# miuda-ai/lele

Hardware: AMD Instinct MI355X
Metric: STFT+mel GB/s (SenseVoice front-end: PCM -> log-mel -> LFR, algorithmic bytes); SenseVoiceSmall-shaped RTF in `sensevoice` (higher is better)
Workload: dtype f32

## Files before the change

lele_amd/csrc/fe_core.h:

```cpp
#pragma once
#include <stdint.h>

#if defined(__HIPCC__)
#define FE_HD __host__ __device__ __forceinline__
#else
#define FE_HD inline
#endif

namespace fe {

constexpr int kNfft = 512;
constexpr int kFrame = 400;
constexpr int kHop = 160;
constexpr int kBins = 257;
constexpr int kLanes = 16;
constexpr int kRegs = 32;
constexpr int kQ = 25;

FE_HD constexpr int rev4(int x) { return ((x & 1) << 3) | ((x & 2) << 1) | ((x & 4) >> 1) | ((x & 8) >> 3); }
FE_HD constexpr int rev5(int x) {
    return ((x & 1) << 4) | ((x & 2) << 2) | (x & 4) | ((x & 8) >> 2) | ((x & 16) >> 4);
}
FE_HD constexpr int tw_off(int s) { return (1 << (s - 1)) - 1; }

FE_HD float fmul(float a, float b) { return a * b; }
FE_HD float fadd(float a, float b) { return a + b; }
FE_HD float fsub(float a, float b) { return a - b; }
FE_HD float ffma(float a, float b, float c) { return __builtin_fmaf(a, b, c); }

#if defined(__HIPCC__) && defined(__HIP_DEVICE_COMPILE__)
typedef float cf __attribute__((ext_vector_type(2)));
FE_HD cf cmk(float re, float im) { return (cf){re, im}; }
FE_HD cf cadd(cf a, cf b) { return a + b; }
FE_HD cf csub(cf a, cf b) { return a - b; }
FE_HD cf cmulv(cf a, cf b) { return a * b; }
FE_HD cf cfmav(cf a, cf b, cf c) { return __builtin_elementwise_fma(a, b, c); }
FE_HD cf cswap(cf a) { return a.yx; }
FE_HD cf cxx(cf a) { return a.xx; }
#else
struct cf {
    float x, y;
};
FE_HD cf cmk(float re, float im) { return cf{re, im}; }
FE_HD cf cadd(cf a, cf b) { return cf{a.x + b.x, a.y + b.y}; }
FE_HD cf csub(cf a, cf b) { return cf{a.x - b.x, a.y - b.y}; }
FE_HD cf cmulv(cf a, cf b) { return cf{a.x * b.x, a.y * b.y}; }
FE_HD cf cfmav(cf a, cf b, cf c) { return cf{__builtin_fmaf(a.x, b.x, c.x), __builtin_fmaf(a.y, b.y, c.y)}; }
FE_HD cf cswap(cf a) { return cf{a.y, a.x}; }
FE_HD cf cxx(cf a) { return cf{a.x, a.x}; }
#endif

struct Tw {
    cf w, wn;
};
FE_HD Tw make_tw(float wr, float wi) { return Tw{cmk(wr, wi), cmk(-wi, wi)}; }

FE_HD cf tw_mul_fma(const Tw& t, cf o) { return cfmav(cxx(t.w), o, cmulv(t.wn, cswap(o))); }

FE_HD void bfly_fma(const Tw& tw, cf& e, cf& o) {
    cf t = tw_mul_fma(tw, o);
    cf n = csub(e, t);
    e = cadd(e, t);
    o = n;
}
FE_HD void bfly_scalar(float wr, float wi, cf& e, cf& o) {
    float tr = fsub(fmul(wr, o.x), fmul(wi, o.y));
    float ti = fadd(fmul(wr, o.y), fmul(wi, o.x));
    cf t = cmk(tr, ti);
    cf n = csub(e, t);
    e = cadd(e, t);
    o = n;
}
FE_HD void bfly_fma(float wr, float wi, float& er, float& ei, float& o_r, float& oi) {
    cf e = cmk(er, ei), o = cmk(o_r, oi);
    bfly_fma(make_tw(wr, wi), e, o);
    er = e.x;
    ei = e.y;
    o_r = o.x;
    oi = o.y;
}
FE_HD void bfly_scalar(float wr, float wi, float& er, float& ei, float& o_r, float& oi) {
    cf e = cmk(er, ei), o = cmk(o_r, oi);
    bfly_scalar(wr, wi, e, o);
    er = e.x;
    ei = e.y;
    o_r = o.x;
    oi = o.y;
}

template <typename TW>
FE_HD void phase_a(cf* a, const TW& tw_re, const TW& tw_im) {
#pragma unroll
    for (int r = 0; r < kRegs; r += 2) bfly_scalar(tw_re[tw_off(1)], tw_im[tw_off(1)], a[r], a[r + 1]);
#pragma unroll
    for (int b = 0; b < kRegs; b += 4) {
#pragma unroll
        for (int k = 0; k < 2; ++k) bfly_scalar(tw_re[tw_off(2) + k], tw_im[tw_off(2) + k], a[b + k], a[b + 2 + k]);
    }
#pragma unroll
    for (int s = 3; s <= 5; ++s) {
        const int half = 1 << (s - 1);
#pragma unroll
        for (int b = 0; b < kRegs; b += 2 * half) {
#pragma unroll
            for (int k = 0; k < half; ++k)
                bfly_fma(make_tw(tw_re[tw_off(s) + k], tw_im[tw_off(s) + k]), a[b + k], a[b + half + k]);
        }
    }
}

template <typename TW>
FE_HD void phase_a_fast(const float* x, cf* a, const TW& tw_re, const TW& tw_im) {
    float s1[kRegs];
#pragma unroll
    for (int r = 0; r < kRegs; r += 2) {
        if (rev5(r + 1) >= kQ) {
            s1[r] = x[r];
            s1[r + 1] = x[r];
        } else {
            s1[r] = fadd(x[r], x[r + 1]);
            s1[r + 1] = fsub(x[r], x[r + 1]);
        }
    }
    {
        const float wr = tw_re[tw_off(2) + 1], wi = tw_im[tw_off(2) + 1];
#pragma unroll
        for (int b = 0; b < kRegs; b += 4) {
            a[b] = cmk(fadd(s1[b], s1[b + 2]), 0.0f);
            a[b + 2] = cmk(fsub(s1[b], s1[b + 2]), 0.0f);
            const float tr = fmul(wr, s1[b + 3]);
            const float ti = fmul(wi, s1[b + 3]);
            a[b + 1] = cmk(fadd(s1[b + 1], tr), ti);
            a[b + 3] = cmk(fsub(s1[b + 1], tr), -ti);
        }
    }
#pragma unroll
    for (int b = 0; b < kRegs; b += 8) {
#pragma unroll
        for (int k = 0; k < 4; ++k) {
            const float wr = tw_re[tw_off(3) + k], wi = tw_im[tw_off(3) + k];
            if ((k & 1) == 0) {
                const float e = a[b + k].x, o = a[b + 4 + k].x;
                const float tr = fmul(wr, o);
                const float ti = fmul(wi, o);
                a[b + k] = cmk(fadd(e, tr), ti);
                a[b + 4 + k] = cmk(fsub(e, tr), -ti);
            } else {
                bfly_fma(make_tw(wr, wi), a[b + k], a[b + 4 + k]);
            }
        }
    }
#pragma unroll
    for (int s = 4; s <= 5; ++s) {
        const int half = 1 << (s - 1);
#pragma unroll
        for (int b = 0; b < kRegs; b += 2 * half) {
#pragma unroll
            for (int k = 0; k < half; ++k)
                bfly_fma(make_tw(tw_re[tw_off(s) + k], tw_im[tw_off(s) + k]), a[b + k], a[b + half + k]);
        }
    }
}

template <typename TWF>
FE_HD void phase_b(cf* b, int c, int rho, const TWF& twf, float* re256) {
#pragma unroll
    for (int s = 6; s <= 8; ++s) {
        const int hv = 1 << (s - 6);
#pragma unroll
        for (int k = 0; k < hv; ++k) {
            const cf w = twf(tw_off(s) + k * 32 + rho * 16 + c);
            const Tw tw = make_tw(w.x, w.y);
#pragma unroll
            for (int base = 0; base < 16; base += 2 * hv) bfly_fma(tw, b[base + k], b[base + hv + k]);
        }
    }
#pragma unroll
    for (int k = 0; k < 8; ++k) {
        const cf w = twf(tw_off(9) + k * 32 + rho * 16 + c);
        const cf t = tw_mul_fma(make_tw(w.x, w.y), b[8 + k]);
        if (k == 0) *re256 = fsub(b[0].x, t.x);
        b[k] = cadd(b[k], t);
    }
}

FE_HD float power(float re, float im) { return fadd(fmul(re, re), fmul(im, im)); }
FE_HD float power(cf z) {
    cf sq = cmulv(z, z);
    return fadd(sq.x, sq.y);
}

constexpr int kXchgPitch = 17;
FE_HD constexpr int xchg_slot(int v, int c) { return v * kXchgPitch + c; }

}
```

lele_amd/csrc/frontend.hip:

```cpp
#include <type_traits>
#include "common.h"
#include "fe_core.h"

#include <math.h>

#include <algorithm>

using namespace lele;

namespace {

constexpr int kMaxMelRounds = 8;

struct FeDev {
    const float* tw_re;
    const float* tw_im;
    const float2* tw;
    const float* window;
    const float* melw;
    const int* mel_start;
    const int* mel_step_off;
    int mel_rounds;
    int mel_steps;
    int n_mels;
// ... 97 lines not shown

__device__ __forceinline__ const float* fe_const_table(const float* t, int pass) {
    auto c = (const __attribute__((address_space(4))) float*)t;
    asm("" : "+s"(c) : "s"(pass));
    return (const float*)c;
}

template <int MODE>
__device__ __forceinline__ float lane_rot_prev(float v, int p) {
    if (MODE == 1) {
        return __builtin_bit_cast(float,
                                  __builtin_amdgcn_update_dpp(0, __builtin_bit_cast(int, v), 0x121, 0xf, 0xf, true));
    } else {
        return __shfl(v, (p + 15) & 15, 16);
    }
}

constexpr int kStdMelLen[5] = {3, 4, 6, 10, 17};
constexpr int kStdMelOff[6] = {0, 3, 7, 13, 23, 40};

template <int MODE, bool STDMEL, bool FUSED, int PASSES, bool LOWREG, class Blk>
__device__ __forceinline__ void fe_main_body(const float* __restrict__ pcm, int64_t utt_stride,
                                             int64_t num_frames, int64_t t_lfr,
                                             const float* __restrict__ means, const FeDev& tb,
                                             float* __restrict__ out, float* __restrict__ logmel_out,
                                             int aligned16, float* s_melw, Blk bl) {
    constexpr int FR = 16 * PASSES;
    constexpr int kRows = FR + 2;
    constexpr int kXFloats = FUSED ? (kRows * kSumPitch > 4 * kWaveLdsFloats ? kRows * kSumPitch : 4 * kWaveLdsFloats)
                                   : 4 * kWaveLdsFloats;
    __shared__ float2 s_tw[LOWREG ? 480 : 512];
    __shared__ __attribute__((aligned(16))) float s_x[kXFloats];
    __shared__ float s_mean[64];
    __shared__ int s_mstart[16 * (STDMEL ? 5 : kMaxMelRounds)];
    __shared__ int s_moff[kMaxMelRounds + 1];
    constexpr int kTwBase = LOWREG ? 31 : 0;

    const int lane = threadIdx.x & 63, wave = threadIdx.x >> 6;
    const int g = lane >> 4, p = lane & 15;
    constexpr int kVecPerRow = fe::kHop / 4;
    constexpr int kVecs = kRows * kVecPerRow;
    constexpr int kIters = (kVecs + 255) / 256;
    constexpr bool kTwDma = FUSED && !LOWREG;
    const bool tile_dma = FUSED && !LOWREG && aligned16 && tb.tile_dma;
    float4 st[FUSED ? kIters : 1];
    if constexpr (FUSED) {
        const float* run = pcm + (int64_t)bl.y() * utt_stride + (int64_t)bl.x() * FR * fe::kHop;
        const int64_t rem64 = utt_stride - (int64_t)bl.x() * FR * fe::kHop;
        const int rem = (int)(rem64 < (1 << 20) ? rem64 : (1 << 20));
        if (tile_dma) {
            constexpr int kSlotsPerRow = kSumPitch / 4;
            constexpr int kDma = (FR - 1 + 2) * kSlotsPerRow + (fe::kFrame - 2 * fe::kHop) / 4;
            constexpr int kDmaInstr = (kDma + 63) / 64;
            static_assert(kDmaInstr * 64 * 4 <= kXFloats, "the tile DMA stays inside s_x");
            auto* tile_lds = (__attribute__((address_space(3))) char*)s_x;
            static_assert(kSlotsPerRow == 41 && kDmaInstr * 64 * 1599 < (1 << 24), "i / 41 == (i * 1599) >> 16 for every slot");
            const unsigned last = 4u * (unsigned)rem - 16u;
            const int wave_s = __builtin_amdgcn_readfirstlane(wave);
#pragma unroll
            for (int u = 0; 4 * u < kDmaInstr; ++u) {
                const unsigned i = 256u * u + threadIdx.x;
                const unsigned ob = 16u * (i - ((i * 1599u) >> 16));
                if (4 * u + 3 < kDmaInstr || 4 * u + wave_s < kDmaInstr)
                    fe_dma16(reinterpret_cast<const char*>(run) + (ob < last ? ob : last), tile_lds + (4 * u + wave_s) * 1024);
            }
        }
        if (kTwDma && wave == 3) {
            auto* tw_lds = (__attribute__((address_space(3))) char*)s_tw;
#pragma unroll
            for (int k = 0; k < 4; ++k)
                fe_dma16(reinterpret_cast<const char*>(tb.tw) + 1024 * k + 16 * lane, tw_lds + 1024 * k);
        }
        if (!tile_dma) {
#pragma unroll
            for (int u = 0; u < kIters; ++u) {
                const int idx = u * 256 + (int)threadIdx.x;
                int o = 4 * idx;
                if (o + 3 >= rem) o = aligned16 ? ((rem - 4) & ~3) : (rem - 4);
                const float* src = run + o;
                if (aligned16)
                    st[u] = *reinterpret_cast<const float4*>(src);
                else
                    st[u] = make_float4(src[0], src[1], src[2], src[3]);
            }
        }
    }
    if (!kTwDma)
        for (int i = threadIdx.x; i < 511 - kTwBase; i += 256) s_tw[i] = tb.tw[i + kTwBase];
    if (!STDMEL)
        for (int i = threadIdx.x; i < tb.mel_steps * 16; i += 256) s_melw[i] = tb.melw[i];
    if (threadIdx.x < tb.mel_rounds * 16) s_mstart[threadIdx.x] = tb.mel_start[threadIdx.x];
    if (threadIdx.x <= tb.mel_rounds) s_moff[threadIdx.x] = tb.mel_step_off[threadIdx.x];
    if (FUSED) {
        if (!tile_dma) {
#pragma unroll
            for (int u = 0; u < kIters; ++u) {
                const int idx = u * 256 + (int)threadIdx.x;
                if (idx < kVecs) {
                    const int row = idx / kVecPerRow, c = idx - row * kVecPerRow;
                    *reinterpret_cast<float4*>(&s_x[row * kSumPitch + 4 * c]) = st[u];
                }
            }
        }
        __builtin_amdgcn_s_waitcnt(0x0F70);
        __syncthreads();
    }
    const int h = fe::rev4(p);
    float* xw = s_x + wave * kWaveLdsFloats;
    float* xf = xw + g * kFrameXchgFloats;
    const float* base = pcm + (int64_t)bl.y() * utt_stride;
    const float* mean_u = means + (int64_t)bl.y() * num_frames;
    const int d_out = tb.n_mels * tb.lfr_m;
    float* out_u = out ? out + (int64_t)bl.y() * t_lfr * d_out : nullptr;
    float* lm_u = logmel_out ? logmel_out + (int64_t)bl.y() * num_frames * tb.n_mels : nullptr;

    float win[fe::kQ];
    if (!LOWREG) {
#pragma unroll
        for (int q = 0; q < fe::kQ; ++q) win[q] = tb.window[p + 16 * q];
    }

    float xr[fe::kQ];
    float mean_next = 0.0f;
    auto issue_loads = [&](int pass) {
        const int64_t f = (int64_t)bl.x() * FR + wave * (4 * PASSES) + pass * 4 + g;
        const int64_t fc = f < num_frames ? f : 0;
        const float* src = base + fc * fe::kHop + p;
        if (!FUSED) mean_next = mean_u[fc];
#pragma unroll
        for (int q = 0; q < fe::kQ; ++q) xr[q] = src[16 * q];
    };
    issue_loads(0);
    if (FUSED) {
        if (wave == 0 && lane < FR) {
            float sum = 0.0f;
#pragma unroll
            for (int seg = 0; seg < 3; ++seg) {
                const float* rowp = &s_x[(lane + seg) * kSumPitch];
                const int nvec = seg < 2 ? kVecPerRow : (fe::kFrame - 2 * fe::kHop) / 4;
#pragma unroll 10
                for (int k = 0; k < nvec; ++k) {
                    const float4 r = *reinterpret_cast<const float4*>(rowp + 4 * k);
                    sum = __builtin_fmaf(r.x, 32768.0f, sum);
                    sum = __builtin_fmaf(r.y, 32768.0f, sum);
                    sum = __builtin_fmaf(r.z, 32768.0f, sum);
                    sum = __builtin_fmaf(r.w, 32768.0f, sum);
                }
            }
            s_mean[lane] = sum / (float)fe::kFrame;
        }
    }
    __syncthreads();

    auto run_pass = [&](int pass, auto load_next_c) {
        constexpr bool load_next = decltype(load_next_c)::value;
        const int64_t f = (int64_t)bl.x() * FR + wave * (4 * PASSES) + pass * 4 + g;
        const bool valid = f < num_frames;
        const float mean = FUSED ? s_mean[wave * (4 * PASSES) + pass * 4 + g] : mean_next;
        if (LOWREG) {
            int off = 0;
            asm volatile("" : "+v"(off));
#pragma unroll
            for (int q = 0; q < fe::kQ; ++q) win[q] = tb.window[p + 16 * q + off];
        }

        float v[fe::kQ];
        const float neg_mean = -mean;
#pragma unroll
        for (int q = 0; q < fe::kQ; ++q) v[q] = __builtin_fmaf(xr[q], 32768.0f, neg_mean);
        if (load_next) issue_loads(pass + 1);
        float xin[fe::kRegs];
#pragma unroll
        for (int r = 0; r < fe::kRegs; ++r) xin[r] = 0.0f;
        float k97;
        asm("v_mov_b32 %0, 0x3f7851ec" : "=v"(k97));
#pragma unroll
        for (int q = 0; q < fe::kQ; ++q) {
            const float send = (p == 15 && q > 0) ? v[q > 0 ? q - 1 : 0] : v[q];
            const float prev = lane_rot_prev<MODE>(send, p);
            float y = fe::fsub(v[q], fe::fmul(k97, prev));
            if (q == 0) y = (p == 0) ? v[0] : y;
            xin[fe::rev5(q)] = fe::fmul(y, win[q]);
        }

        fe::cf a[fe::kRegs];
        fe::phase_a_fast(xin, a, fe_const_table(tb.tw_re, pass), fe_const_table(tb.tw_im, pass));

        float pw[2][8];
        float p256 = 0.0f;
#pragma unroll
        for (int rho = 0; rho < 2; ++rho) {
            __builtin_amdgcn_wave_barrier();
#pragma unroll
            for (int cc = 0; cc < 16; ++cc) {
                const int slot = fe::xchg_slot(h, cc);
                *reinterpret_cast<float2*>(xf + 2 * slot) = make_float2(a[rho * 16 + cc].x, a[rho * 16 + cc].y);
            }
            __builtin_amdgcn_wave_barrier();
            fe::cf bq[16];
#pragma unroll
            for (int vv = 0; vv < 16; ++vv) {
                const float2 t = *reinterpret_cast<const float2*>(xf + 2 * fe::xchg_slot(vv, p));
                bq[vv] = fe::cmk(t.x, t.y);
            }
            __builtin_amdgcn_wave_barrier();
            float re256 = 0.0f;
            fe::phase_b(bq, p, rho, [&](int i) { const float2 w = s_tw[i - kTwBase]; return fe::cmk(w.x, w.y); }, &re256);
            if (rho == 0) p256 = re256;
#pragma unroll
            for (int vv = 0; vv < 8; ++vv) {
                fe::cf z = bq[vv];
                if (vv == 0 && rho == 0) z = fe::cmk(z.x, (p == 0) ? 0.0f : z.y);
                pw[rho][vv] = fe::power(z);
            }
        }
        float* prow = xw + g * kPStride;
        __builtin_amdgcn_wave_barrier();
#pragma unroll
        for (int rho = 0; rho < 2; ++rho)
#pragma unroll
            for (int vv = 0; vv < 8; ++vv) prow[(2 * vv + rho) * 16 + p] = pw[rho][vv];
        if (p == 0) prow[256] = fe::power(p256, 0.0f);
        __builtin_amdgcn_wave_barrier();

        const int fi = (int)f, nfr = (int)num_frames, tl = (int)t_lfr;
        const int pad = (tb.lfr_m - 1) / 2;
        const int fp = fi + pad;
        const int b_first = fp % tb.lfr_n, i_first = fp / tb.lfr_n;

        float vals[STDMEL ? 5 : kMaxMelRounds];
#pragma unroll
        for (int rd = 0; rd < (STDMEL ? 5 : kMaxMelRounds); ++rd) {
            vals[rd] = 0.0f;
            if (!STDMEL && rd >= tb.mel_rounds) continue;
            const int m = rd * 16 + p;
            const int start = s_mstart[m];
            const float* pp = prow + start;
            float acc = 0.0f;
            if (STDMEL) {
                const float* wp = tb.melw + kStdMelOff[rd < 5 ? rd : 0] * 16 + p;
                float w[17];
#pragma unroll
                for (int t = 0; t < 17; ++t)
                    if (t < kStdMelLen[rd < 5 ? rd : 0]) w[t] = wp[t * 16];
#pragma unroll
                for (int t = 0; t < 17; ++t)
                    if (t < kStdMelLen[rd < 5 ? rd : 0]) acc = fe::fadd(acc, fe::fmul(w[t], pp[t]));
            } else {
                const int t0 = s_moff[rd], t1 = s_moff[rd + 1];
                const float* wp = s_melw + t0 * 16 + p;
                const int lim = 256 - start;
#pragma unroll 4
                for (int t = 0; t < t1 - t0; ++t) {
                    const float pv = pp[t < lim ? t : lim];
                    acc = fe::fadd(acc, fe::fmul(wp[t * 16], pv));
                }
            }
            {
                const float l2 = __builtin_amdgcn_logf(fmaxf(acc, 1e-5f));
                const float hi = __builtin_bit_cast(float, 0x3f317217u), lo = __builtin_bit_cast(float, 0x3377d1cfu);
                const float r = fe::fmul(l2, hi);
                vals[rd] = fe::fadd(r, fe::ffma(l2, lo, fe::ffma(l2, hi, -r)));
            }
        }
        if (valid) {
            constexpr int kR = STDMEL ? 5 : kMaxMelRounds;
            auto put = [&](float* dst) {
#pragma unroll
                for (int rd = 0; rd < kR; ++rd)
                    if (rd * 16 + p < tb.n_mels) __builtin_nontemporal_store(vals[rd], &dst[rd * 16]);
            };
            if (lm_u) put(lm_u + (int64_t)fi * tb.n_mels + p);
            if (out_u) {
                int i = i_first;
                for (int b = b_first; b < tb.lfr_m && i >= 0; b += tb.lfr_n, --i)
                    if (i < tl) put(out_u + i * d_out + b * tb.n_mels + p);
                if (fi == 0) {
                    for (int i2 = 0; i2 * tb.lfr_n - pad < 0 && i2 < tl; ++i2)
                        for (int b = 0; b < tb.lfr_m && i2 * tb.lfr_n + b - pad < 0; ++b)
                            put(out_u + i2 * d_out + b * tb.n_mels + p);
                }
                if (fi == nfr - 1) {
                    for (int i2 = tl - 1; i2 >= 0 && i2 * tb.lfr_n + (tb.lfr_m - 1) - pad > fi; --i2)
                        for (int b = tb.lfr_m - 1; b >= 0 && i2 * tb.lfr_n + b - pad > fi; --b)
                            put(out_u + i2 * d_out + b * tb.n_mels + p);
                }
            }
        }
        __builtin_amdgcn_wave_barrier();
    };
#pragma unroll 1
    for (int pass = 0; pass + 1 < PASSES; ++pass) run_pass(pass, std::true_type{});
    run_pass(PASSES - 1, std::false_type{});
}

template <int MODE, bool STDMEL, bool FUSED>
__global__ __launch_bounds__(256) void fe_main_kernel(const float* __restrict__ pcm, int64_t utt_stride, int64_t num_frames, int64_t t_lfr,
                                                      const float* __restrict__ means, FeDev tb, float* __restrict__ out,
                                                      float* __restrict__ logmel_out, int aligned16) {
    extern __shared__ float s_melw[];
    fe_main_body<MODE, STDMEL, FUSED, 4, false>(pcm, utt_stride, num_frames, t_lfr, means, tb, out, logmel_out, aligned16, s_melw,
                                                GridBlock{});
}

template <int MODE, bool STDMEL>
__global__ __launch_bounds__(256) void fe_seg_main_kernel(const float* __restrict__ pcm, const FeSeg* __restrict__ segs,
                                                          const int* __restrict__ blk_seg, FeDev tb, float* __restrict__ out) {
    extern __shared__ float s_melw[];
    const FeSeg s = segs[blk_seg[blockIdx.x]];
    const float* base = pcm + s.start;
    const int aligned16 = (((uintptr_t)base & 15) == 0) && (s.len % 4 == 0);
    fe_main_body<MODE, STDMEL, true, 4, false>(base, s.len, s.num_frames, s.t_lfr, nullptr, tb, out + s.row0 * (tb.n_mels * tb.lfr_m),
                                               nullptr, aligned16, s_melw, SegBlock{(unsigned)(blockIdx.x - s.block0)});
}
__global__ void fe_generic_mean_kernel(const float* __restrict__ pcm, int64_t rows, int64_t num_frames, int64_t pcm_len, int frame_len, int hop,
                                       float* __restrict__ mean) {
    const int64_t f = (int64_t)blockIdx.x * blockDim.x + threadIdx.x;
    if (f >= rows) return;
    const float* src = pcm + (f / num_frames) * pcm_len + (f % num_frames) * hop;
    float sum = 0.0f;
    int j = 0;
    if ((((uintptr_t)src) & 15) == 0) {
        for (; j + 16 <= frame_len; j += 16) {
            float4 v[4];
#pragma unroll
            for (int u = 0; u < 4; ++u) v[u] = *reinterpret_cast<const float4*>(src + j + 4 * u);
#pragma unroll
            for (int u = 0; u < 4; ++u) {
                sum = sum + v[u].x * 32768.0f;
                sum = sum + v[u].y * 32768.0f;
                sum = sum + v[u].z * 32768.0f;
                sum = sum + v[u].w * 32768.0f;
            }
        }
    }
    for (; j < frame_len; ++j) sum = sum + src[j] * 32768.0f;
    mean[f] = sum / (float)frame_len;
}
__global__ void fe_generic_frame_kernel(const float* __restrict__ pcm, const float* __restrict__ mean,
                                        const float* __restrict__ window, int64_t rows, int64_t num_frames, int64_t pcm_len, int frame_len, int hop,
                                        int n_fft, float* __restrict__ frames) {
    const int64_t total = rows * n_fft;
    for (int64_t i = (int64_t)blockIdx.x * blockDim.x + threadIdx.x; i < total; i += (int64_t)gridDim.x * blockDim.x) {
        const int64_t f = i / n_fft;
        const int j = (int)(i - f * n_fft);
        float v = 0.0f;
        if (j < frame_len) {
            const float* src = pcm + (f / num_frames) * pcm_len + (f % num_frames) * hop;
            const float m = mean[f];
            const float cur = fe::fsub(fe::fmul(src[j], 32768.0f), m);
            float y = cur;
            if (j >= 1) y = fe::fsub(cur, fe::fmul(0.97f, fe::fsub(fe::fmul(src[j - 1], 32768.0f), m)));
            v = fe::fmul(y, window[j]);
        }
        frames[i] = v;
    }
}
__global__ void fe_generic_mel_kernel(const float* __restrict__ power, int64_t num_frames, int n_bins, int n_mels,
                                      const int* __restrict__ mstart, const int* __restrict__ moff,
                                      const float* __restrict__ mw, float* __restrict__ logmel) {
    const int64_t total = num_frames * n_mels;
    for (int64_t i = (int64_t)blockIdx.x * blockDim.x + threadIdx.x; i < total; i += (int64_t)gridDim.x * blockDim.x) {
        const int64_t f = i / n_mels;
        const int m = (int)(i - f * n_mels);
        const float* p = power + f * n_bins + mstart[m];
        float acc = 0.0f;
        for (int t = moff[m]; t < moff[m + 1]; ++t) acc = fe::fadd(acc, fe::fmul(mw[t], p[t - moff[m]]));
        logmel[i] = __logf(fmaxf(acc, 1e-5f));
    }
}
#define FE_PAD(i) ((i) + ((i) >> 5))
__global__ __launch_bounds__(256) void fe_generic_fused_kernel(const float* __restrict__ pcm, int64_t pcm_len, int64_t num_frames, int frame_len,
                                                               int hop, int n, int log2n, int fpb, const float* __restrict__ window,
                                                               const float* __restrict__ tw_re_g, const float* __restrict__ tw_im_g, int n_mels,
                                                               const int* __restrict__ mstart, const int* __restrict__ moff,
                                                               const float* __restrict__ mw, const float* __restrict__ means,
                                                               float* __restrict__ logmel) {
    extern __shared__ float gfl[];
    const int nb = n / 2 + 1, span = (fpb - 1) * hop + frame_len;
    float* re = gfl;
    float* im = re + FE_PAD(fpb * n) + 1;
    float* pw = im + FE_PAD(fpb * n) + 1;
    float* sp = pw + fpb * nb;
    float* smean = sp + span;
    const int tid = threadIdx.x;
    const int64_t f0 = (int64_t)blockIdx.x * fpb;
    const int nfr = (int)(num_frames - f0 < fpb ? num_frames - f0 : fpb);
    const float* src = pcm + (int64_t)blockIdx.y * pcm_len + f0 * hop;
    const int have = (nfr - 1) * hop + frame_len;
    for (int i = tid; i < span; i += 256) sp[i] = i < have ? src[i] : 0.0f;
    __syncthreads();
    if (means) {
        if (tid < nfr) smean[tid] = means[(int64_t)blockIdx.y * num_frames + f0 + tid];
    } else if (tid < nfr) {
        const float* fr = sp + tid * hop;
        float sum = 0.0f;
        int j = 0;
        for (; j + 16 <= frame_len; j += 16) {
            float v[16];
#pragma unroll
            for (int u = 0; u < 16; ++u) v[u] = fr[j + u];
#pragma unroll
            for (int u = 0; u < 16; ++u) sum = sum + v[u] * 32768.0f;
        }
        for (; j < frame_len; ++j) sum = sum + fr[j] * 32768.0f;
        smean[tid] = sum / (float)frame_len;
    }
    __syncthreads();
    for (int i = tid; i < fpb * n; i += 256) {
        const int f = i >> log2n, j = i & (n - 1);
        float v = 0.0f;
        if (j < frame_len && f < nfr) {
            const float* fr = sp + f * hop;
            const float m = smean[f];
            const float cur = fe::fsub(fe::fmul(fr[j], 32768.0f), m);
            float y = cur;
            if (j >= 1) y = fe::fsub(cur, fe::fmul(0.97f, fe::fsub(fe::fmul(fr[j - 1], 32768.0f), m)));
            v = fe::fmul(y, window[j]);
        }
        const int r = (int)(__brev((unsigned)j) >> (32 - log2n));
        re[FE_PAD(f * n + r)] = v;
        im[FE_PAD(f * n + r)] = 0.0f;
    }
    __syncthreads();
    for (int s0 = 0; s0 < log2n;) {
        const int R = log2n - s0 >= 3 ? 3 : log2n - s0, h = 1 << s0, gsz = 1 << R, groups = n >> R;
        for (int idx = tid; idx < fpb * groups; idx += 256) {
            const int f = idx / groups, g = idx - f * groups;
            const int lo = g & (h - 1), base = f * n + ((g >> s0) << (s0 + R)) + lo;
            float xr[8], xi[8];
#pragma unroll
            for (int j = 0; j < 8; ++j)
                if (j < gsz) xr[j] = re[FE_PAD(base + j * h)], xi[j] = im[FE_PAD(base + j * h)];
#pragma unroll
            for (int r = 0; r < 3; ++r) {
                if (r >= R) break;
                const int half = h << r, off = half - 1;
#pragma unroll
                for (int j = 0; j < 8; ++j) {
                    if (j >= gsz || (j >> r) & 1) continue;
                    const int k = lo + (j & ((1 << r) - 1)) * h;
                    const float wr = tw_re_g[off + k], wi = tw_im_g[off + k];
                    if (half >= 4)
                        fe::bfly_fma(wr, wi, xr[j], xi[j], xr[j + (1 << r)], xi[j + (1 << r)]);
                    else
// ... 62 lines not shown
    FeDev dev{};
    std::vector<void*> allocs;
    DevTables seg_tables;
    bool profiling = false;
    std::vector<hipEvent_t> events;
    size_t events_used = 0;
};

namespace {

static const float PI_F = 3.14159265358979323846264338327950288f;

void host_hann(int64_t size, std::vector<float>& w) {
    w.resize(size);
    if (size == 1) w[0] = 1.0f;
    for (int64_t n = 0; size > 1 && n < size; ++n) w[n] = 0.5f * (1.0f - cosf(2.0f * PI_F * (float)n / (float)(size - 1)));
}

void host_twiddles(int64_t n, std::vector<float>& re, std::vector<float>& im) {
    re.clear();
    im.clear();
    for (int64_t size = 2; size <= n; size *= 2) {
        int64_t half = size / 2, step = n / size;
        for (int64_t k = 0; k < half; ++k) {
            float angle = -2.0f * PI_F * (float)(k * step) / (float)n;
            re.push_back(cosf(angle));
            im.push_back(sinf(angle));
        }
    }
}

float hz_to_mel(float hz) { return 2595.0f * log10f(1.0f + hz / 700.0f); }
float mel_to_hz(float mel) { return 700.0f * (powf(10.0f, mel / 2595.0f) - 1.0f); }

void host_dense_mel(float sr, int64_t n_fft, int64_t n_mels, float f_min, float f_max, float* bank) {
    const int64_t n_freqs = n_fft / 2 + 1;
    const float mel_min = hz_to_mel(f_min), mel_max = hz_to_mel(f_max);
    const float mel_step = (mel_max - mel_min) / (float)(n_mels + 1);
    std::vector<float> hz(n_mels + 2), ff(n_freqs);
    for (int64_t i = 0; i < n_mels + 2; ++i) hz[i] = mel_to_hz(mel_min + (float)i * mel_step);
    for (int64_t i = 0; i < n_freqs; ++i) ff[i] = (float)i * sr / (float)n_fft;
    for (int64_t i = 0; i < n_mels; ++i) {
        const float fl = hz[i], fc = hz[i + 1], fr = hz[i + 2];
        for (int64_t j = 0; j < n_freqs; ++j) {
            const float f = ff[j];
            float val = 0.0f;
            if (f > fl && f < fc)
                val = (f - fl) / (fc - fl);
            else if (f >= fc && f < fr)
                val = (fr - f) / (fr - fc);
            bank[i * n_freqs + j] = val;
        }
    }
}

void host_sparse_mel(float sr, int64_t n_fft, int64_t n_mels, float f_min, std::vector<int>& start,
                     std::vector<std::vector<float>>& w) {
    const int64_t n_freqs = n_fft / 2 + 1;
    std::vector<float> bank((size_t)n_mels * n_freqs);
    host_dense_mel(sr, n_fft, n_mels, f_min, sr / 2.0f, bank.data());
    start.assign(n_mels, 0);
    w.assign(n_mels, {});
    for (int64_t i = 0; i < n_mels; ++i) {
        const float* row = bank.data() + i * n_freqs;
        int64_t s = 0;
        while (s < n_freqs && row[s] == 0.0f) ++s;
        int64_t e = n_freqs;
        while (e > s && row[e - 1] == 0.0f) --e;
        if (s < e) {
            start[i] = (int)s;
            w[i].assign(row + s, row + e);
        }
    }
}

template <typename T>
int upload(LeleFrontend* fe, const std::vector<T>& v, const T** out) {
    void* d = nullptr;
    size_t bytes = std::max<size_t>(v.size() * sizeof(T), 16);
    LELE_HIP_CHECK(hipMalloc(&d, bytes));
    fe->allocs.push_back(d);
    if (!v.empty()) LELE_HIP_CHECK(hipMemcpy(d, v.data(), v.size() * sizeof(T), hipMemcpyHostToDevice));
    *out = (const T*)d;
    return 0;
}

}

extern "C" {

int lele_hip_hann_window(int64_t size, float* out) {
    LELE_REQUIRE(size >= 0 && (out || size == 0), "hann_window: bad argument");
    std::vector<float> w;
    host_hann(size, w);
    if (size) memcpy(out, w.data(), (size_t)size * 4);
    return 0;
}
float lele_hip_hz_to_mel_htk(float hz) { return hz_to_mel(hz); }
float lele_hip_mel_to_hz_htk(float mel) { return mel_to_hz(mel); }
int lele_hip_mel_filterbank(float sample_rate, int64_t n_fft, int64_t n_mels, float f_min, int32_t has_f_max, float f_max, float* out) {
    LELE_REQUIRE(n_fft >= 0 && n_mels >= 0 && (out || n_mels == 0), "mel_filterbank: bad argument");
    if (n_mels) host_dense_mel(sample_rate, n_fft, n_mels, f_min, has_f_max ? f_max : sample_rate / 2.0f, out);
    return 0;
}


int lele_hip_frontend_create(LeleCtx* ctx, const LeleFeatureConfig* cfg, LeleFrontend** out) {
    LELE_REQUIRE(ctx && cfg && out, "frontend_create: NULL argument");
    LELE_REQUIRE(cfg->sample_rate > 0 && cfg->n_mels > 0 && cfg->lfr_m > 0 && cfg->lfr_n > 0,
                 "frontend_create: invalid FeatureConfig");
    LELE_HIP_CHECK(hipSetDevice(ctx->device));
    LeleFrontend* fe = new LeleFrontend();
    fe->ctx = ctx;
    fe->cfg = *cfg;
    fe->frame_len = (int64_t)((float)cfg->sample_rate * cfg->frame_length_ms / 1000.0f);
    fe->n_fft = fe->frame_len > 400 ? 1024 : 512;
    fe->hop_len = (int64_t)((float)cfg->sample_rate * cfg->frame_shift_ms / 1000.0f);
    fe->fast = (fe->frame_len == fe::kFrame && fe->hop_len == fe::kHop && fe->n_fft == fe::kNfft &&
                cfg->n_mels <= 16 * kMaxMelRounds);
    if (!fe->fast) {
        if (fe->frame_len < 1 || fe->hop_len < 1 || fe->frame_len > fe->n_fft) {
            const long long fl = (long long)fe->frame_len, hl = (long long)fe->hop_len, nf = (long long)fe->n_fft;
            delete fe;
            set_error("frontend_create: frame_len=%lld hop_len=%lld do not fit fft_len=%lld (the reference panics here)", fl, hl, nf);
            return 3;
        }
        std::vector<float> gwin;
        host_hann(fe->frame_len, gwin);
        std::vector<int> gstart;
        std::vector<std::vector<float>> gw;
        host_sparse_mel((float)cfg->sample_rate, fe->n_fft, cfg->n_mels, 20.0f, gstart, gw);
        std::vector<int> goff(cfg->n_mels + 1, 0);
        std::vector<float> gflat;
        for (int64_t m = 0; m < cfg->n_mels; ++m) {
            goff[m] = (int)gflat.size();
            gflat.insert(gflat.end(), gw[m].begin(), gw[m].end());
        }
        goff[cfg->n_mels] = (int)gflat.size();
        int rc = 0;
        rc |= upload(fe, gwin, &fe->g_window);
        rc |= upload(fe, gstart, &fe->g_mstart);
        rc |= upload(fe, goff, &fe->g_moff);
        rc |= upload(fe, gflat, &fe->g_mw);
        if (rc) {
            lele_hip_frontend_destroy(fe);
            return rc;
        }
        *out = fe;
        return 0;
    }
    std::vector<float> win, twr, twi;
    host_hann(fe->frame_len, win);
    host_twiddles(fe->n_fft, twr, twi);
    LELE_REQUIRE(twr[0] == 1.0f && twi[0] == 0.0f && twr[1] == 1.0f && twi[1] == 0.0f,
                 "frontend_create: unexpected twiddle table head");
    std::vector<float2> tw(512, make_float2(0.f, 0.f));
    for (size_t i = 0; i < twr.size(); ++i) tw[i] = make_float2(twr[i], twi[i]);
    twr.resize(512, 0.0f);
    twi.resize(512, 0.0f);
    std::vector<int> mstart;
    std::vector<std::vector<float>> mw;
    host_sparse_mel((float)cfg->sample_rate, fe->n_fft, cfg->n_mels, 20.0f, mstart, mw);
    FeDev& d = fe->dev;
    d.n_mels = (int)cfg->n_mels;
    d.lfr_m = (int)cfg->lfr_m;
    d.lfr_n = (int)cfg->lfr_n;
    d.mel_rounds = (int)((cfg->n_mels + 15) / 16);
    std::vector<int> start_pad(d.mel_rounds * 16, 0);
    std::vector<float> melw;
    std::vector<int> step_off(d.mel_rounds + 1, 0);
    int off = 0;
    for (int rd = 0; rd < d.mel_rounds; ++rd) {
        size_t maxlen = 0;
        for (int pm = 0; pm < 16; ++pm) {
            int m = rd * 16 + pm;
            if (m < cfg->n_mels) {
                start_pad[m] = mstart[m];
                maxlen = std::max(maxlen, mw[m].size());
            }
        }
        step_off[rd] = off;
        for (size_t t = 0; t < maxlen; ++t)
            for (int pm = 0; pm < 16; ++pm) {
                int m = rd * 16 + pm;
                melw.push_back((m < cfg->n_mels && t < mw[m].size()) ? mw[m][t] : 0.0f);
            }
        off += (int)maxlen;
    }
    step_off[d.mel_rounds] = off;
    d.mel_steps = off;
    fe->std_mel = (d.mel_rounds == 5 && cfg->n_mels == 80);
    for (int rd = 0; fe->std_mel && rd < 5; ++rd) {
        if (step_off[rd] != kStdMelOff[rd] || step_off[rd + 1] != kStdMelOff[rd + 1]) fe->std_mel = false;
        for (int pm = 0; pm < 16; ++pm)
            if (start_pad[rd * 16 + pm] + kStdMelLen[rd] - 1 > 256) fe->std_mel = false;
    }
    if (lab_env("LELE_HIP_FE_GENERIC_MEL")) fe->std_mel = false;
    int rc = 0;
    rc |= upload(fe, twr, &d.tw_re);
    rc |= upload(fe, twi, &d.tw_im);
    rc |= upload(fe, tw, &d.tw);
    rc |= upload(fe, win, &d.window);
    rc |= upload(fe, melw, &d.melw);
    rc |= upload(fe, start_pad, &d.mel_start);
    rc |= upload(fe, step_off, &d.mel_step_off);
    if (rc) {
        lele_hip_frontend_destroy(fe);
        return rc;
    }
    const char* env = lab_env("LELE_HIP_FE_DPP");
    fe->dpp_mode = env ? atoi(env) : 1;
    const char* envf = lab_env("LELE_HIP_FE_FUSED");
    fe->fused = envf ? atoi(envf) != 0 : true;
    const char* envd = getenv("LELE_HIP_FE_TILE_DMA");
    d.tile_dma = envd && *envd ? atoi(envd) != 0 : 1;
    *out = fe;
    return 0;
}

int lele_hip_frontend_destroy(LeleFrontend* fe) {
    if (!fe) return 0;
    (void)hipStreamSynchronize(fe->ctx->stream);
    for (void* p : fe->allocs) (void)hipFree(p);
    fe->seg_tables.release();
    for (hipEvent_t e : fe->events) (void)hipEventDestroy(e);
    delete fe;
    return 0;
}

int lele_hip_frontend_out_rows(const LeleFrontend* fe, int64_t pcm_len, int64_t* rows, int64_t* cols,
                               int64_t* num_frames) {
    LELE_REQUIRE(fe, "frontend_out_rows: fe is NULL");
    int64_t nf = 0, t = 0;
    if (pcm_len >= fe->frame_len) {
        nf = (pcm_len - fe->frame_len) / fe->hop_len + 1;
        t = (nf + fe->cfg.lfr_n - 1) / fe->cfg.lfr_n;
    }
    if (rows) *rows = t;
    if (cols) *cols = fe->cfg.n_mels * fe->cfg.lfr_m;
    if (num_frames) *num_frames = nf;
    return 0;
}

static int ilog2_i(int n) {
    int l = 0;
    while ((1 << (l + 1)) <= n) ++l;
    return l;
}
static int fe_generic(LeleFrontend* fe, const float* dpcm, int64_t batch, int64_t pcm_len, int64_t nf, int64_t t_lfr, int64_t cols,
                      float* outp, bool want_logmel, void* dmean) {
    LeleCtx* ctx = fe->ctx;
    const int64_t bins = fe->n_fft / 2 + 1, nm = fe->cfg.n_mels;
    if (fe->fused && fe->n_fft <= 4096 && fe->frame_len <= fe->n_fft && batch <= 65535) {
        const int n = (int)fe->n_fft;
        int fpb = n <= 512 ? 4 : n <= 1024 ? 2 : 1;
        if (const char* e = lab_env("LELE_HIP_FE_FPB")) fpb = std::max(1, atoi(e));
        const size_t padded = (size_t)fpb * n + (((size_t)fpb * n) >> 5) + 1;
        const size_t lds = (2 * padded + (size_t)fpb * bins + (size_t)(fpb - 1) * fe->hop_len + fe->frame_len + fpb) * 4;
        if (lds <= 96 * 1024) {
            const float *twr = nullptr, *twi = nullptr;
            LELE_TRY(fft_twiddles(ctx, n, &twr, &twi));
            LELE_HIP_CHECK(ensure_dyn_lds(reinterpret_cast<const void*>(fe_generic_fused_kernel), (int)lds));
            const int64_t per_utt_lm = nf * nm * 4;
            const int64_t ubf = want_logmel ? batch : std::max<int64_t>(1, std::min<int64_t>(batch, (int64_t(1) << 28) / std::max<int64_t>(per_utt_lm, 1)));
            void* glm = nullptr;
            if (!want_logmel) LELE_TRY(ctx->arena_alloc((size_t)ubf * nf * nm * 4, &glm));
            for (int64_t u = 0; u < batch; u += ubf) {
                const int64_t nu = std::min<int64_t>(ubf, batch - u);
                const float* up = (const float*)dpcm + u * pcm_len;
                float* lm = want_logmel ? outp + u * nf * nm : (float*)glm;
                hipLaunchKernelGGL(fe_generic_mean_kernel, dim3((unsigned)((nu * nf + 63) / 64)), dim3(64), 0, ctx->stream, up, nu * nf, nf, pcm_len,
                                   (int)fe->frame_len, (int)fe->hop_len, (float*)dmean);
                hipLaunchKernelGGL(fe_generic_fused_kernel, dim3((unsigned)((nf + fpb - 1) / fpb), (unsigned)nu), dim3(256), lds, ctx->stream, up,
                                   pcm_len, nf, (int)fe->frame_len, (int)fe->hop_len, n, ilog2_i(n), fpb, fe->g_window, twr, twi, (int)nm,
                                   fe->g_mstart, fe->g_moff, fe->g_mw, (const float*)dmean, lm);
                if (!want_logmel) {
                    dim3 lg((unsigned)std::max<int64_t>(1, std::min<int64_t>((t_lfr * cols + 255) / 256, 8192)), (unsigned)nu);
                    hipLaunchKernelGGL(fe_generic_lfr_kernel, lg, dim3(256), 0, ctx->stream, (const float*)lm, nf, nm, fe->cfg.lfr_m,
                                       fe->cfg.lfr_n, t_lfr, outp + u * t_lfr * cols);
                }
            }
            LELE_HIP_CHECK(hipGetLastError());
            return 0;
        }
    }
    const int64_t per_utt = nf * (4 + fe->n_fft * 4 + bins * 4 + nm * 4);
    const int64_t ub = std::max<int64_t>(1, std::min<int64_t>(std::min<int64_t>(batch, 65535), (int64_t(1) << 28) / std::max<int64_t>(per_utt, 1)));
    void *gm = nullptr, *gf = nullptr, *gp = nullptr, *gl = nullptr;
    LELE_TRY(ctx->arena_alloc((size_t)ub * nf * 4, &gm));
    LELE_TRY(ctx->arena_alloc((size_t)ub * nf * fe->n_fft * 4, &gf));
    LELE_TRY(ctx->arena_alloc((size_t)ub * nf * bins * 4, &gp));
    if (!want_logmel) LELE_TRY(ctx->arena_alloc((size_t)ub * nf * nm * 4, &gl));
    auto blocks = [](int64_t n) { return dim3((unsigned)std::max<int64_t>(1, std::min<int64_t>((n + 255) / 256, 8192))); };
    for (int64_t u = 0; u < batch; u += ub) {
        const int64_t nu = std::min<int64_t>(ub, batch - u), rows = nu * nf;
        const float* up = (const float*)dpcm + u * pcm_len;
        float* lm = want_logmel ? outp + u * nf * nm : (float*)gl;
        hipLaunchKernelGGL(fe_generic_mean_kernel, dim3((unsigned)((rows + 63) / 64)), dim3(64), 0, ctx->stream, up, rows, nf, pcm_len,
                           (int)fe->frame_len, (int)fe->hop_len, (float*)gm);
        hipLaunchKernelGGL(fe_generic_frame_kernel, blocks(rows * fe->n_fft), dim3(256), 0, ctx->stream, up, (const float*)gm,
                           fe->g_window, rows, nf, pcm_len, (int)fe->frame_len, (int)fe->hop_len, (int)fe->n_fft, (float*)gf);
        LELE_TRY(fft_rows_power(ctx, (const float*)gf, rows, fe->n_fft, (float*)gp));
        hipLaunchKernelGGL(fe_generic_mel_kernel, blocks(rows * nm), dim3(256), 0, ctx->stream, (const float*)gp, rows, (int)bins,
                           (int)nm, fe->g_mstart, fe->g_moff, fe->g_mw, lm);
        if (!want_logmel) {
            dim3 lg = blocks(t_lfr * cols);
            lg.y = (unsigned)nu;
            hipLaunchKernelGGL(fe_generic_lfr_kernel, lg, dim3(256), 0, ctx->stream, (const float*)lm, nf, nm,
                               fe->cfg.lfr_m, fe->cfg.lfr_n, t_lfr, outp + u * t_lfr * cols);
        }
    }
    LELE_HIP_CHECK(hipGetLastError());
    return 0;
}

static int fe_run(LeleFrontend* fe, const LeleTensor* pcm, int64_t batch, int64_t pcm_len, LeleBuf* out,
                  bool want_logmel, int64_t* out_shape, int32_t* out_rank) {
    LeleCtx* ctx = fe->ctx;
    LELE_HIP_CHECK(hipSetDevice(ctx->device));
    LELE_REQUIRE(pcm->dtype == LELE_F32, "frontend: pcm must be f32");
    int64_t t_lfr = 0, cols = 0, nf = 0;
    lele_hip_frontend_out_rows(fe, pcm_len, &t_lfr, &cols, &nf);
    if (nf == 0 || batch == 0) {
        out->bytes = 0;
        if (out_rank) *out_rank = 0;
        return 0;
    }
    LELE_TRY(ctx->arena_reset());
    const void* dpcm = nullptr;
    LELE_TRY(ctx->dev_ptr(pcm, &dpcm));
    void* dmean = nullptr;
    LELE_TRY(ctx->get_scratch((size_t)batch * nf * sizeof(float), &dmean));
    const size_t out_elems = want_logmel ? (size_t)batch * nf * fe->cfg.n_mels : (size_t)batch * t_lfr * cols;
    LELE_TRY(out->reserve(out_elems * sizeof(float)));
    if (!fe->fast) {
        LELE_TRY(fe_generic(fe, (const float*)dpcm, batch, pcm_len, nf, t_lfr, cols, (float*)out->data, want_logmel, dmean));
        if (want_logmel) {
            if (batch == 1) return set_shape(out_shape, out_rank, {nf, fe->cfg.n_mels});
            return set_shape(out_shape, out_rank, {batch, nf, fe->cfg.n_mels});
        }
        return 0;
    }
    const int aligned16 = ((uintptr_t)dpcm % 16 == 0) && (pcm_len % 4 == 0);
    dim3 grid((unsigned)((nf + 63) / 64), (unsigned)batch);
    hipEvent_t* ev = nullptr;
    if (fe->profiling) {
        if (fe->events_used + 3 > fe->events.size()) {
            for (int i = 0; i < 3; ++i) {
                hipEvent_t e;
                LELE_HIP_CHECK(hipEventCreate(&e));
                fe->events.push_back(e);
            }
        }
        ev = &fe->events[fe->events_used];
        fe->events_used += 3;
        LELE_HIP_CHECK(hipEventRecord(ev[0], ctx->stream));
    }
    if (!fe->fused)
        hipLaunchKernelGGL(fe_frame_sum_kernel, grid, dim3(64), 0, ctx->stream, (const float*)dpcm, pcm_len, pcm_len, nf,
                           (float*)dmean, aligned16);
    if (ev) LELE_HIP_CHECK(hipEventRecord(ev[1], ctx->stream));
    const size_t mel_lds = (size_t)fe->dev.mel_steps * 16 * sizeof(float);
    float* o = want_logmel ? nullptr : (float*)out->data;
    float* lm = want_logmel ? (float*)out->data : nullptr;
#define FE_LAUNCH(MODE, STD, FUS)                                                                                     \
    hipLaunchKernelGGL((fe_main_kernel<MODE, STD, FUS>), grid, dim3(256), mel_lds, ctx->stream, (const float*)dpcm, \
                       pcm_len, nf, t_lfr, (const float*)dmean, fe->dev, o, lm, aligned16)
#define FE_LAUNCH2(MODE, STD) \
    do {                      \
        if (fe->fused)        \
            FE_LAUNCH(MODE, STD, true); \
        else                  \
            FE_LAUNCH(MODE, STD, false); \
    } while (0)
    if (fe->dpp_mode == 1) {
        if (fe->std_mel) FE_LAUNCH2(1, true); else FE_LAUNCH2(1, false);
    } else {
        if (fe->std_mel) FE_LAUNCH2(0, true); else FE_LAUNCH2(0, false);
    }
#undef FE_LAUNCH2
#undef FE_LAUNCH
    LELE_HIP_CHECK(hipGetLastError());
    if (ev) LELE_HIP_CHECK(hipEventRecord(ev[2], ctx->stream));
    if (want_logmel) {
        if (batch == 1) return set_shape(out_shape, out_rank, {nf, fe->cfg.n_mels});
        return set_shape(out_shape, out_rank, {batch, nf, fe->cfg.n_mels});
    }
    return 0;
}

int lele_hip_frontend_compute(LeleFrontend* fe, const LeleTensor* pcm, LeleBuf* out, int64_t* out_shape,
                              int32_t* out_rank) {
    LELE_REQUIRE(fe && pcm && out, "frontend_compute: NULL argument");
    const int64_t n = numel(pcm);
    LELE_TRY(fe_run(fe, pcm, 1, n, out, false, out_shape, out_rank));
    if (out->bytes == 0) return 0;
    int64_t t = 0, cols = 0;
    lele_hip_frontend_out_rows(fe, n, &t, &cols, nullptr);
    return set_shape(out_shape, out_rank, {t, cols});
}

int lele_hip_frontend_compute_batch(LeleFrontend* fe, const LeleTensor* pcm, LeleBuf* out, int64_t* out_shape,
                                    int32_t* out_rank) {
    LELE_REQUIRE(fe && pcm && out, "frontend_compute_batch: NULL argument");
    LELE_REQUIRE(pcm->rank == 2, "frontend_compute_batch: pcm must be [batch, pcm_len]");
    const int64_t batch = pcm->shape[0], n = pcm->shape[1];
    LELE_TRY(fe_run(fe, pcm, batch, n, out, false, out_shape, out_rank));
    if (out->bytes == 0) return 0;
    int64_t t = 0, cols = 0;
    lele_hip_frontend_out_rows(fe, n, &t, &cols, nullptr);
    return set_shape(out_shape, out_rank, {batch, t, cols});
}

int lele_hip_frontend_logmel(LeleFrontend* fe, const LeleTensor* pcm, LeleBuf* out, int64_t* out_shape,
                             int32_t* out_rank) {
    LELE_REQUIRE(fe && pcm && out, "frontend_logmel: NULL argument");
    if (pcm->rank == 2) return fe_run(fe, pcm, pcm->shape[0], pcm->shape[1], out, true, out_shape, out_rank);
    return fe_run(fe, pcm, 1, numel(pcm), out, true, out_shape, out_rank);
}

struct SegLayout {
    const LeleFrontend* fe;
    const int64_t* starts;
    const int64_t* lengths;
    int64_t count;
    const int64_t* rows;
};
static void build_seg_table(const void* arg, std::vector<char>& blob) {
    const SegLayout& L = *(const SegLayout*)arg;
    std::vector<FeSeg> segs;
    std::vector<int> blk;
    for (int64_t i = 0; i < L.count; ++i) {
        int64_t t = 0, nf = 0;
        lele_hip_frontend_out_rows(L.fe, L.lengths[i], &t, nullptr, &nf);
        if (nf == 0) continue;
        const int64_t nb = (nf + 63) / 64;
        segs.push_back(FeSeg{L.starts[i], L.lengths[i], nf, t, L.rows[i], (int64_t)blk.size()});
        blk.insert(blk.end(), (size_t)nb, (int)segs.size() - 1);
    }
    blob.resize(segs.size() * sizeof(FeSeg) + blk.size() * sizeof(int));
    memcpy(blob.data(), segs.data(), segs.size() * sizeof(FeSeg));
    memcpy(blob.data() + segs.size() * sizeof(FeSeg), blk.data(), blk.size() * sizeof(int));
}

int lele_hip_frontend_compute_segments(LeleFrontend* fe, const LeleTensor* pcm, const int64_t* starts, const int64_t* lengths, int64_t count,
                                       LeleBuf* out, int64_t* row_offsets, int64_t* out_shape, int32_t* out_rank) {
    LELE_REQUIRE(fe && pcm && out && row_offsets, "frontend_compute_segments: NULL argument");
    LELE_REQUIRE(count >= 0 && (count == 0 || (starts && lengths)), "frontend_compute_segments: bad segment arrays (count %lld)",
                 (long long)count);
    LELE_REQUIRE(pcm->dtype == LELE_F32 && pcm->rank == 1, "frontend_compute_segments: pcm must be f32 [N]");
    const int64_t n = pcm->shape[0];
    for (int64_t i = 0; i < count; ++i)
        LELE_REQUIRE(starts[i] >= 0 && lengths[i] >= 0 && starts[i] <= n - lengths[i],
                     "frontend_compute_segments: segment %lld (start %lld, length %lld) lies outside the %lld samples of pcm", (long long)i,
                     (long long)starts[i], (long long)lengths[i], (long long)n);
    int64_t cols = fe->cfg.n_mels * fe->cfg.lfr_m, blocks = 0, max_nf = 0;
    row_offsets[0] = 0;
    for (int64_t i = 0; i < count; ++i) {
        int64_t t = 0, nf = 0;
        lele_hip_frontend_out_rows(fe, lengths[i], &t, nullptr, &nf);
        row_offsets[i + 1] = row_offsets[i] + t;
        blocks += (nf + 63) / 64;
        max_nf = std::max(max_nf, nf);
    }
    const int64_t rows = row_offsets[count];
    if (rows == 0) {
        out->bytes = 0;
        if (out_rank) *out_rank = 0;
        return 0;
    }
    LELE_REQUIRE(blocks < (int64_t(1) << 31), "frontend_compute_segments: %lld blocks exceed the grid", (long long)blocks);
    LeleCtx* ctx = fe->ctx;
    LELE_HIP_CHECK(hipSetDevice(ctx->device));
    LELE_TRY(ctx->arena_reset());
    const void* dpcm = nullptr;
    LELE_TRY(ctx->dev_ptr(pcm, &dpcm));
    LELE_TRY(out->reserve((size_t)rows * cols * sizeof(float)));
    float* o = (float*)out->data;
    if (!fe->fast) {
        void* dmean = nullptr;
        LELE_TRY(ctx->get_scratch((size_t)max_nf * sizeof(float), &dmean));
        const size_t mark = ctx->arena_used;
        for (int64_t i = 0; i < count; ++i) {
            int64_t t = 0, nf = 0;
            lele_hip_frontend_out_rows(fe, lengths[i], &t, nullptr, &nf);
            if (nf == 0) continue;
            LELE_TRY(fe_generic(fe, (const float*)dpcm + starts[i], 1, lengths[i], nf, t, cols, o + row_offsets[i] * cols, false, dmean));
            ctx->arena_used = mark;
        }
        return set_shape(out_shape, out_rank, {rows, cols});
    }
    std::string key((size_t)count * 16, '\0');
    memcpy(&key[0], starts, (size_t)count * 8);
    memcpy(&key[(size_t)count * 8], lengths, (size_t)count * 8);
    const SegLayout lay{fe, starts, lengths, count, row_offsets};
    const void* table = nullptr;
    LELE_TRY(fe->seg_tables.get(ctx, std::move(key), build_seg_table, &lay, &table));
    int64_t nseg = 0;
    for (int64_t i = 0; i < count; ++i) nseg += lengths[i] >= fe->frame_len;
    const FeSeg* dsegs = (const FeSeg*)table;
    const int* dblk = (const int*)(dsegs + nseg);
    const size_t mel_lds = (size_t)fe->dev.mel_steps * 16 * sizeof(float);
#define FE_SEG_LAUNCH(MODE, STD)                                                                                                 \
    hipLaunchKernelGGL((fe_seg_main_kernel<MODE, STD>), dim3((unsigned)blocks), dim3(256), mel_lds, ctx->stream, (const float*)dpcm, \
                       dsegs, dblk, fe->dev, o)
    if (fe->dpp_mode == 1) {
        if (fe->std_mel) FE_SEG_LAUNCH(1, true); else FE_SEG_LAUNCH(1, false);
    } else {
        if (fe->std_mel) FE_SEG_LAUNCH(0, true); else FE_SEG_LAUNCH(0, false);
    }
#undef FE_SEG_LAUNCH
    LELE_HIP_CHECK(hipGetLastError());
    return set_shape(out_shape, out_rank, {rows, cols});
}

int lele_hip_frontend_set_profiling(LeleFrontend* fe, int on) {
    LELE_REQUIRE(fe, "frontend_set_profiling: fe is NULL");
    fe->profiling = on != 0;
    fe->events_used = 0;
    return 0;
}

int lele_hip_frontend_profile_read(LeleFrontend* fe, float* sum_kernel_ms, float* main_kernel_ms, int64_t* runs) {
    LELE_REQUIRE(fe, "frontend_profile_read: fe is NULL");
    LELE_HIP_CHECK(hipStreamSynchronize(fe->ctx->stream));
    double a = 0, b = 0;
    const size_t n = fe->events_used / 3;
    for (size_t i = 0; i < n; ++i) {
        float m0 = 0, m1 = 0;
        LELE_HIP_CHECK(hipEventElapsedTime(&m0, fe->events[3 * i], fe->events[3 * i + 1]));
        LELE_HIP_CHECK(hipEventElapsedTime(&m1, fe->events[3 * i + 1], fe->events[3 * i + 2]));
        a += m0;
        b += m1;
    }
    if (sum_kernel_ms) *sum_kernel_ms = n ? (float)(a / n) : 0.f;
    if (main_kernel_ms) *main_kernel_ms = n ? (float)(b / n) : 0.f;
    if (runs) *runs = (int64_t)n;
    fe->events_used = 0;
    return 0;
}

}
```

Before: 1885.

## Trim FFT trivial twiddles, hoist mel starts, and strength-reduce LFR output addressing

Stage 4/5 butterflies with k=0 now use a plain add/sub because that twiddle is 1, and a host check confirms the table entries. Mel start indices for the standard layout are loaded from shared memory once into registers instead of once per pass. Mel dot products load all powers before the multiply-add chain. LFR output offsets are kept as 32-bit byte offsets that advance by strength reduction across passes instead of being recomputed with div/mod each pass, with new host guards that cap the output size so 32-bit offsets cannot overflow. Together these cut ALU and integer work per frame in the fused front-end kernel.

After: 1933 (median of 6 runs). 2.5% higher.

```diff
diff --git a/lele_amd/csrc/fe_core.h b/lele_amd/csrc/fe_core.h
--- a/lele_amd/csrc/fe_core.h
+++ b/lele_amd/csrc/fe_core.h
@@ -155,8 +155,13 @@
         const int half = 1 << (s - 1);
 #pragma unroll
         for (int b = 0; b < kRegs; b += 2 * half) {
-#pragma unroll
-            for (int k = 0; k < half; ++k)
+            {
+                const cf e = a[b], o = a[b + half];
+                a[b] = cadd(e, o);
+                a[b + half] = csub(e, o);
+            }
+#pragma unroll
+            for (int k = 1; k < half; ++k)
                 bfly_fma(make_tw(tw_re[tw_off(s) + k], tw_im[tw_off(s) + k]), a[b + k], a[b + half + k]);
         }
     }
diff --git a/lele_amd/csrc/frontend.hip b/lele_amd/csrc/frontend.hip
--- a/lele_amd/csrc/frontend.hip
+++ b/lele_amd/csrc/frontend.hip
@@ -273,10 +273,37 @@
     }
     __syncthreads();
 
+    int mstart[5] = {0, 0, 0, 0, 0};
+    if (STDMEL) {
+#pragma unroll
+        for (int rd = 0; rd < 5; ++rd) mstart[rd] = s_mstart[rd * 16 + p];
+    }
+
+    const int f_first = (int)(bl.x() * FR) + wave * (4 * PASSES) + g;
+    const int nfr = (int)num_frames, tl = (int)t_lfr;
+    const int pad = (tb.lfr_m - 1) / 2;
+    const unsigned blk_bytes = 4u * (unsigned)tb.n_mels, row_bytes = 4u * (unsigned)d_out;
+    auto target_off = [&](int i, int b) { return (unsigned)i * row_bytes + (unsigned)b * blk_bytes + 4u * (unsigned)p; };
+    int lfr_b = (f_first + pad) % tb.lfr_n, lfr_i = (f_first + pad) / tb.lfr_n;
+    unsigned lfr_o = target_off(lfr_i, lfr_b);
+    auto next_targets = [&]() {
+        lfr_b += 4;
+        if (tb.lfr_n >= 4) {
+            const bool carry = lfr_b >= tb.lfr_n;
+            lfr_b -= carry ? tb.lfr_n : 0;
+            lfr_i += carry ? 1 : 0;
+            lfr_o += carry ? 4u * blk_bytes + row_bytes - (unsigned)tb.lfr_n * blk_bytes : 4u * blk_bytes;
+        } else {
+            lfr_i += lfr_b / tb.lfr_n;
+            lfr_b = lfr_b % tb.lfr_n;
+            lfr_o = target_off(lfr_i, lfr_b);
+        }
+    };
+
     auto run_pass = [&](int pass, auto load_next_c) {
         constexpr bool load_next = decltype(load_next_c)::value;
-        const int64_t f = (int64_t)bl.x() * FR + wave * (4 * PASSES) + pass * 4 + g;
-        const bool valid = f < num_frames;
+        const int fi = f_first + pass * 4;
+        const bool valid = fi < nfr;
         const float mean = FUSED ? s_mean[wave * (4 * PASSES) + pass * 4 + g] : mean_next;
         if (LOWREG) {
             int off = 0;
@@ -344,29 +371,30 @@
         if (p == 0) prow[256] = fe::power(p256, 0.0f);
         __builtin_amdgcn_wave_barrier();
 
-        const int fi = (int)f, nfr = (int)num_frames, tl = (int)t_lfr;
-        const int pad = (tb.lfr_m - 1) / 2;
-        const int fp = fi + pad;
-        const int b_first = fp % tb.lfr_n, i_first = fp / tb.lfr_n;
-
         float vals[STDMEL ? 5 : kMaxMelRounds];
 #pragma unroll
         for (int rd = 0; rd < (STDMEL ? 5 : kMaxMelRounds); ++rd) {
             vals[rd] = 0.0f;
             if (!STDMEL && rd >= tb.mel_rounds) continue;
             const int m = rd * 16 + p;
-            const int start = s_mstart[m];
+            const int start = STDMEL ? mstart[rd < 5 ? rd : 0] : s_mstart[m];
             const float* pp = prow + start;
             float acc = 0.0f;
             if (STDMEL) {
                 const float* wp = tb.melw + kStdMelOff[rd < 5 ? rd : 0] * 16 + p;
-                float w[17];
+                float w[17], pv[17];
 #pragma unroll
                 for (int t = 0; t < 17; ++t)
                     if (t < kStdMelLen[rd < 5 ? rd : 0]) w[t] = wp[t * 16];
 #pragma unroll
                 for (int t = 0; t < 17; ++t)
-                    if (t < kStdMelLen[rd < 5 ? rd : 0]) acc = fe::fadd(acc, fe::fmul(w[t], pp[t]));
+                    if (t < kStdMelLen[rd < 5 ? rd : 0]) pv[t] = pp[t];
+#pragma unroll
+                for (int t = 0; t < 17; ++t)
+                    if (t < kStdMelLen[rd < 5 ? rd : 0]) {
+                        const float wp0 = fe::fmul(w[t], pv[t]);
+                        acc = t == 0 ? wp0 : fe::fadd(acc, wp0);
+                    }
             } else {
                 const int t0 = s_moff[rd], t1 = s_moff[rd + 1];
                 const float* wp = s_melw + t0 * 16 + p;
@@ -386,32 +414,36 @@
         }
         if (valid) {
             constexpr int kR = STDMEL ? 5 : kMaxMelRounds;
-            auto put = [&](float* dst) {
+            auto put = [&](float* dst_u, unsigned off) {
+                float* dst = reinterpret_cast<float*>(reinterpret_cast<char*>(dst_u) + off);
 #pragma unroll
                 for (int rd = 0; rd < kR; ++rd)
-                    if (rd * 16 + p < tb.n_mels) __builtin_nontemporal_store(vals[rd], &dst[rd * 16]);
+                    if (STDMEL || rd * 16 + p < tb.n_mels)
+                        __builtin_nontemporal_store(vals[rd], &dst[rd * 16]);
             };
-            if (lm_u) put(lm_u + (int64_t)fi * tb.n_mels + p);
+            if (lm_u) put(lm_u, (unsigned)fi * blk_bytes + 4u * (unsigned)p);
             if (out_u) {
-                int i = i_first;
-                for (int b = b_first; b < tb.lfr_m && i >= 0; b += tb.lfr_n, --i)
-                    if (i < tl) put(out_u + i * d_out + b * tb.n_mels + p);
+                int i = lfr_i;
+                unsigned o = lfr_o;
+                for (int b = lfr_b; b < tb.lfr_m && i >= 0; b += tb.lfr_n, --i, o += (unsigned)tb.lfr_n * blk_bytes - row_bytes)
+                    if (i < tl) put(out_u, o);
                 if (fi == 0) {
                     for (int i2 = 0; i2 * tb.lfr_n - pad < 0 && i2 < tl; ++i2)
-                        for (int b = 0; b < tb.lfr_m && i2 * tb.lfr_n + b - pad < 0; ++b)
-                            put(out_u + i2 * d_out + b * tb.n_mels + p);
+                        for (int b = 0; b < tb.lfr_m && i2 * tb.lfr_n + b - pad < 0; ++b) put(out_u, target_off(i2, b));
                 }
                 if (fi == nfr - 1) {
                     for (int i2 = tl - 1; i2 >= 0 && i2 * tb.lfr_n + (tb.lfr_m - 1) - pad > fi; --i2)
-                        for (int b = tb.lfr_m - 1; b >= 0 && i2 * tb.lfr_n + b - pad > fi; --b)
-                            put(out_u + i2 * d_out + b * tb.n_mels + p);
+                        for (int b = tb.lfr_m - 1; b >= 0 && i2 * tb.lfr_n + b - pad > fi; --b) put(out_u, target_off(i2, b));
                 }
             }
         }
         __builtin_amdgcn_wave_barrier();
     };
 #pragma unroll 1
-    for (int pass = 0; pass + 1 < PASSES; ++pass) run_pass(pass, std::true_type{});
+    for (int pass = 0; pass + 1 < PASSES; ++pass) {
+        run_pass(pass, std::true_type{});
+        next_targets();
+    }
     run_pass(PASSES - 1, std::false_type{});
 }
 
@@ -780,8 +812,8 @@
     std::vector<float> win, twr, twi;
     host_hann(fe->frame_len, win);
     host_twiddles(fe->n_fft, twr, twi);
-    LELE_REQUIRE(twr[0] == 1.0f && twi[0] == 0.0f && twr[1] == 1.0f && twi[1] == 0.0f,
-                 "frontend_create: unexpected twiddle table head");
+    for (int i : {0, 1, fe::tw_off(4), fe::tw_off(5)})
+        LELE_REQUIRE(twr[i] == 1.0f && twi[i] == 0.0f, "frontend_create: unexpected twiddle table entry %d", i);
     std::vector<float2> tw(512, make_float2(0.f, 0.f));
     for (size_t i = 0; i < twr.size(); ++i) tw[i] = make_float2(twr[i], twi[i]);
     twr.resize(512, 0.0f);
@@ -969,6 +1001,8 @@
         }
         return 0;
     }
+    LELE_REQUIRE((want_logmel ? nf * fe->cfg.n_mels : t_lfr * cols) < (int64_t(1) << 30),
+                 "frontend: the features of one utterance (%lld frames) exceed 4 GiB", (long long)nf);
     const int aligned16 = ((uintptr_t)dpcm % 16 == 0) && (pcm_len % 4 == 0);
     dim3 grid((unsigned)((nf + 63) / 64), (unsigned)batch);
     hipEvent_t* ev = nullptr;
@@ -1098,6 +1132,8 @@
         return 0;
     }
     LELE_REQUIRE(blocks < (int64_t(1) << 31), "frontend_compute_segments: %lld blocks exceed the grid", (long long)blocks);
+    LELE_REQUIRE(!fe->fast || (max_nf + fe->cfg.lfr_n - 1) / fe->cfg.lfr_n * cols < (int64_t(1) << 30),
+                 "frontend_compute_segments: the features of one segment (%lld frames) exceed 4 GiB", (long long)max_nf);
     LeleCtx* ctx = fe->ctx;
     LELE_HIP_CHECK(hipSetDevice(ctx->device));
     LELE_TRY(ctx->arena_reset());
```
